# nyu-systems/Grendel-GS

Hardware: AMD Instinct MI355X
Metric: training iters/sec (fwd+bwd) (higher is better)
Workload: dtype f32

## Files before the change

grendel-gs_amd/csrc/binning.hip:

```cpp
#include "common.h"

#include <atomic>
#include <chrono>
#include <cstdlib>
#include <cstring>
#include <mutex>

#include "radix.h"
#ifndef GSR_EMIT_DECODE_BATCH
#define GSR_EMIT_DECODE_BATCH 2
#endif
#include "binning_persist.h"
#include "binning_rows.h"

namespace {

__global__ void __launch_bounds__(SCAN_THREADS)
scan_gather_lookback_kernel(const uint32_t *__restrict__ src, int packed,
                            const uint32_t *__restrict__ idx, uint32_t *__restrict__ out, uint32_t *__restrict__ out2,
                            long long n, unsigned long long *__restrict__ state, uint32_t *__restrict__ ticket, int nb,
                            uint32_t *__restrict__ host_total, uint32_t seq,
                            const unsigned long long *__restrict__ early) {
    __shared__ uint32_t smem[4];
    __shared__ uint32_t s_bid;
// ... 510 lines not shown
}

int prepare_lookback(const PrepCall &c, uint32_t *ticket) {
    const int P = c.P;
    hipStream_t stream = c.stream;
    const PrepLayout L = prep_layout(P, c.width, c.height);
    const int gx = (c.width + GSR_BLOCK_X - 1) / GSR_BLOCK_X, gy = (c.height + GSR_BLOCK_Y - 1) / GSR_BLOCK_Y;
    char *base = reinterpret_cast<char *>(c.prep);
    uint32_t *tt = reinterpret_cast<uint32_t *>(base + L.tt);
    uint32_t *kA = reinterpret_cast<uint32_t *>(base + L.kA), *vA = reinterpret_cast<uint32_t *>(base + L.vA);
    uint32_t *kB = reinterpret_cast<uint32_t *>(base + L.kB), *vB = reinterpret_cast<uint32_t *>(base + L.vB);
    uint32_t *offsets = reinterpret_cast<uint32_t *>(base + L.offsets);
    TileRect *rects = reinterpret_cast<TileRect *>(base + L.rects);
    char *ctrl = base + L.ctrl;

    GSR_HIP(hipMemsetAsync(base + L.early, 0, (L.ctrl - L.early) + L.C.total, stream));
    const RadixPlan plan = radix_plan(0, 32);
    uint32_t *host_total = nullptr;
    uint32_t seq = 0;
    int rc = total_slot(&host_total, &seq);
    if (rc) return rc;
    uint32_t *tile_hist = yx_path(gx, gy) ? reinterpret_cast<uint32_t *>(base + L.thist) : nullptr;
    const int blocks = gsr_div_up(P, TC_THREADS) < TC_BLOCKS ? gsr_div_up(P, TC_THREADS) : TC_BLOCKS;
    hipLaunchKernelGGL(touch_count_kernel, dim3(blocks), dim3(TC_THREADS), 0, stream, P, gx, gy,
                       reinterpret_cast<const float2 *>(c.means2D), c.depths, c.radii,
                       reinterpret_cast<const float4 *>(c.conic_opacity), c.compute_locally, plan, tt, kA, vA, rects,
                       reinterpret_cast<uint32_t *>(ctrl + L.C.ghist), tile_hist,
                       reinterpret_cast<int32_t *>(base + L.hull), tile_hist ? tile_cull_on(gx * gy) : 0,
                       reinterpret_cast<unsigned long long *>(base + L.early), host_total, seq,
                       reinterpret_cast<uint4 *>(c.zero_ptr), c.zero_bytes / 16);
    int in_first = 1;
    rc = radix_sort_pairs(kA, vA, kB, vB, P, plan, ctrl, L.C, &in_first, stream, nullptr);
    if (rc) return rc;
    uint32_t *sorted_ids = in_first ? vA : vB;
    if (!in_first) {
        hipLaunchKernelGGL(copy_u32_kernel, dim3(gsr_div_up(P, GSR_ONE_DIM_BLOCK)), dim3(GSR_ONE_DIM_BLOCK), 0, stream,
                           (long long)P, vB, vA);
        sorted_ids = vA;
    }
    if (g_tie_order.load(std::memory_order_relaxed) == 1)
        hipLaunchKernelGGL(depth_tie_fixup_kernel, dim3(gsr_div_up(P, GSR_ONE_DIM_BLOCK)), dim3(GSR_ONE_DIM_BLOCK), 0,
                           stream, (long long)P, in_first ? kA : kB, sorted_ids,
                           reinterpret_cast<const float2 *>(c.means2D));
    const int nbs = gsr_div_up(P, SCAN_TILE);
    hipLaunchKernelGGL(scan_gather_lookback_kernel, dim3(nbs), dim3(SCAN_THREADS), 0, stream, tt,
                       tile_hist ? 1 : 0, sorted_ids, offsets,
                       reinterpret_cast<uint32_t *>(base + L.segoff), (long long)P,
                       reinterpret_cast<unsigned long long *>(ctrl + L.C.scan_state),
                       reinterpret_cast<uint32_t *>(ctrl + L.C.tickets), nbs, (uint32_t *)nullptr, seq,
                       reinterpret_cast<const unsigned long long *>(base + L.early));
    GSR_LAUNCH_CHECK();
    *ticket = seq;
    return 0;
}

int prepare_persistent(const PrepCall &c, uint32_t *ticket) {
    if (!(persist_effective_mode() & PERSIST_P) || g_tie_order.load(std::memory_order_relaxed) != 0) return 1;
    int dev = 0;
    GSR_HIP(hipGetDevice(&dev));
    if (dev < 0 || dev >= 64) return 1;
    PersistCaps caps;
    persist_caps(dev, &caps);
    const int max_tpw = env_cap("GSR_BIN_MAX_TPW", PP_MAX_TPW + 1) <= PP_MAX_TPW ? env_cap("GSR_BIN_MAX_TPW", PP_MAX_TPW + 1) : 1;
    long long nb = radix_blocks(c.P);
    int items = 4;
    if (nb > caps.grid_p && (nb + 1) / 2 <= caps.grid_p) {
        items = 8;
        nb = (nb + 1) / 2;
    }
    const int G = (int)(nb < caps.grid_p ? nb : caps.grid_p);
    if (G <= 0 || nb > (long long)G * max_tpw) return 1;
    const long long admit = persist_admit(dev, c.stream);
    if (admit < 0) return 1;
    const int P = c.P;
    const PrepLayout L = prep_layout(P, c.width, c.height);
    const PersistLayoutP PL = persist_layout_p(G);
    const int gx = (c.width + GSR_BLOCK_X - 1) / GSR_BLOCK_X, gy = (c.height + GSR_BLOCK_Y - 1) / GSR_BLOCK_Y;
    char *base = reinterpret_cast<char *>(c.prep);
    char *ctrl = base + L.ctrl;
    GSR_HIP(hipMemsetAsync(base + L.early, 0, (L.ctrl - L.early) + PL.zero_bytes, c.stream));
    uint32_t *host_total = nullptr;
    uint32_t seq = 0;
    int rc = total_slot(&host_total, &seq);
    if (rc) return rc;
    PrepPersistArgs a{};
    a.P = P; a.gx = gx; a.gy = gy;
    a.means2D = reinterpret_cast<const float2 *>(c.means2D);
    a.depths = c.depths;
    a.radii = c.radii;
    a.conic_opacity = reinterpret_cast<const float4 *>(c.conic_opacity);
    a.mask = c.compute_locally;
    a.tt = reinterpret_cast<uint32_t *>(base + L.tt);
    a.kA = reinterpret_cast<uint32_t *>(base + L.kA); a.vA = reinterpret_cast<uint32_t *>(base + L.vA);
    a.kB = reinterpret_cast<uint32_t *>(base + L.kB); a.vB = reinterpret_cast<uint32_t *>(base + L.vB);
    a.offsets = reinterpret_cast<uint32_t *>(base + L.offsets);
    a.segoff = reinterpret_cast<uint32_t *>(base + L.segoff);
    a.rects = reinterpret_cast<TileRect *>(base + L.rects);
    a.tile_hist = yx_path(gx, gy) ? reinterpret_cast<uint32_t *>(base + L.thist) : nullptr;
    a.cull = a.tile_hist ? tile_cull_on(gx * gy) : 0;
    a.hull_out = reinterpret_cast<int32_t *>(base + L.hull);
    a.early = reinterpret_cast<unsigned long long *>(base + L.early);
    a.zero16 = reinterpret_cast<uint4 *>(c.zero_ptr);
    a.zero16_n = c.zero_bytes / 16;
    const int ngroups = (G + GB_FAN - 1) / GB_FAN;
    a.sync.leaf = reinterpret_cast<uint32_t *>(ctrl + PL.sync);
    a.sync.root = a.sync.leaf + (size_t)ngroups * GB_LEAF_STRIDE;
    a.sync.flags = a.sync.root + GB_LEAF_STRIDE;
    a.tstamp = timeline_buffer(0, G);
    a.grp = reinterpret_cast<uint32_t *>(ctrl + PL.grp);
    a.cnt = reinterpret_cast<uint32_t *>(ctrl + PL.cnt);
    a.wtot = reinterpret_cast<unsigned long long *>(ctrl + PL.wtot);
    a.host_total = host_total;
    a.seq = seq;
    a.done_word = g_persist_done[dev];
    a.done_seq = (uint32_t)admit;
    a.timeout_ticks = 5000000ull;
    a.force_abort = force_abort_env('p') ? 1 : 0;
    if (items == 4) hipLaunchKernelGGL(bin_prepare_persist_kernel<4>, dim3(G), dim3(PP_THREADS), 0, c.stream, a);
    else hipLaunchKernelGGL(bin_prepare_persist_kernel<8>, dim3(G), dim3(PP_THREADS), 0, c.stream, a);
    GSR_LAUNCH_CHECK();
    *ticket = seq;
    return 0;
}
}

namespace {
int prepare_async_impl(int P, int width, int height, const float *means2D, const float *depths, const int32_t *radii,
                       const float *conic_opacity, const uint8_t *compute_locally, void *prep, size_t prep_bytes,
                       uint32_t *ticket, gsr_stream_t stream_, void *zero_ptr, size_t zero_bytes);
}
extern "C" int gsr_bin_prepare_async(int P, int width, int height, const float *means2D, const float *depths,
                                     const int32_t *radii, const float *conic_opacity, const uint8_t *compute_locally,
                                     void *prep, size_t prep_bytes, uint32_t *ticket, gsr_stream_t stream_) {
    return prepare_async_impl(P, width, height, means2D, depths, radii, conic_opacity, compute_locally, prep, prep_bytes,
                              ticket, stream_, nullptr, 0);
}
namespace {
int prepare_async_impl(int P, int width, int height, const float *means2D, const float *depths, const int32_t *radii,
                       const float *conic_opacity, const uint8_t *compute_locally, void *prep, size_t prep_bytes,
                       uint32_t *ticket, gsr_stream_t stream_, void *zero_ptr, size_t zero_bytes) {
    hipStream_t stream = reinterpret_cast<hipStream_t>(stream_);
    if (P < 0 || width <= 0 || height <= 0 || !ticket) return GSR_EINVAL;
    *ticket = 0;
    if (P == 0) return 0;
    if (!means2D || !depths || !radii || !conic_opacity || !compute_locally || !prep) return GSR_EINVAL;
    if (P > RADIX_MAX_N) return GSR_EINVAL;
    if (prep_bytes < prep_layout_full(P, width, height).total) return GSR_ENOSPACE;
    const int gx = (width + GSR_BLOCK_X - 1) / GSR_BLOCK_X, gy = (height + GSR_BLOCK_Y - 1) / GSR_BLOCK_Y;
    if (gx > 0xFFFF || gy > 0xFFFF) return GSR_EINVAL;
    PrepCall c{P, width, height, means2D, depths, radii, conic_opacity, compute_locally, prep, stream, true,
               zero_ptr, zero_bytes};
    {
        int dev0 = 0;
        GSR_HIP(hipGetDevice(&dev0));
        const int fault = persist_fault_check(dev0);
        if (fault) return fault;
    }
    int rc = prepare_persistent(c, ticket);
    if (rc == 1) {
        c.persistent = false;
        rc = prepare_lookback(c, ticket);
    }
    if (rc) return rc;
    int dev = 0;
// ... 423 lines not shown
```

grendel-gs_amd/csrc/binning_persist.h:

```cpp
#pragma once

namespace {

constexpr int TT_SHIFT = 20;
constexpr uint32_t TT_MASK = (1u << TT_SHIFT) - 1u;
constexpr uint32_t GB_ABORT = 0x80000000u;
constexpr int GB_FAN = 32;
constexpr int GB_LEAF_STRIDE = 32;
constexpr uint32_t PAIRS_ABORTED = 0xFFFFFFFFu;

struct GridSync {
    uint32_t *leaf;
    uint32_t *root;
    uint32_t *flags;
};
__host__ __device__ inline size_t grid_sync_words(int G) {
    return (size_t)(2 * ((G + GB_FAN - 1) / GB_FAN) + 1) * GB_LEAF_STRIDE;
}

__device__ __forceinline__ bool grid_barrier_try_abort(const GridSync gs, uint32_t complete) {
    uint32_t r = __hip_atomic_load(gs.root, __ATOMIC_RELAXED, __HIP_MEMORY_SCOPE_AGENT);
    while (true) {
        if (r & GB_ABORT) return true;
        if (r == complete) return false;
// ... 228 lines not shown
    out.xs = (uint32_t)minx | ((uint32_t)maxx << 16);
    out.ys = (uint32_t)miny | ((uint32_t)maxy << 16);
    out.mask = ~0ull;
    if (!cull || w * h > 64) {
        if (dxy) {
            atomicAdd(&dxy[0][minx], h);
            atomicAdd(&dxy[0][maxx], -h);
            atomicAdd(&dxy[1][miny], w);
            atomicAdd(&dxy[1][maxy], -w);
            atomicAdd(&dxy[2][miny], 1);
            atomicAdd(&dxy[2][maxy], -1);
        }
        return (uint32_t)(w * h);
    }
    const unsigned long long mask = gsr_tile_mask(xy, co, minx, miny, maxx, maxy);
    out.mask = mask;
    if (dxy) {
        const unsigned long long rowm = gsr_full_mask(w);
        int prev_cnt = 0, run_a0 = 0, run_len = 0, run_mult = 0;
        for (int r = 0; r < h; r++) {
            unsigned long long bits = (mask >> (r * w)) & rowm;
            const int cnt = __popcll(bits);
            if (cnt != prev_cnt) atomicAdd(&dxy[1][miny + r], cnt - prev_cnt);
            prev_cnt = cnt;
            while (bits) {
                const int a0 = __ffsll((long long)bits) - 1;
                const unsigned long long rest = ~(bits >> a0);
                const int len = rest ? __ffsll((long long)rest) - 1 : 64 - a0;
                if (run_mult && a0 == run_a0 && len == run_len) {
                    run_mult++;
                } else {
                    if (run_mult) {
                        atomicAdd(&dxy[0][minx + run_a0], run_mult);
                        atomicAdd(&dxy[0][minx + run_a0 + run_len], -run_mult);
                    }
                    run_a0 = a0; run_len = len; run_mult = 1;
                }
                bits &= ~(gsr_full_mask(len) << a0);
            }
        }
        if (run_mult) {
            atomicAdd(&dxy[0][minx + run_a0], run_mult);
            atomicAdd(&dxy[0][minx + run_a0 + run_len], -run_mult);
        }
        if (prev_cnt) atomicAdd(&dxy[1][maxy], -prev_cnt);
    }
    return (uint32_t)__popcll(mask);
}

template <int ITEMS, int THREADS>
struct PersistSmem {
    uint16_t wtab[THREADS / 64][RADIX_DIGITS];
    uint32_t gbase[RADIX_DIGITS];
    uint32_t skey[ITEMS * THREADS], sval[ITEMS * THREADS];
    uint32_t scan_tmp[THREADS / 64];
    unsigned long long scan64[THREADS / 64];
    uint32_t flag;
};

template <int ITEMS, int THREADS>
__device__ __forceinline__ void clear_wtab(PersistSmem<ITEMS, THREADS> &sm) {
    uint32_t *p = reinterpret_cast<uint32_t *>(&sm.wtab[0][0]);
    for (int i = threadIdx.x; i < (THREADS / 64) * RADIX_DIGITS / 2; i += THREADS) p[i] = 0u;
}

template <int ITEMS, int THREADS>
__device__ __forceinline__ void count_wave_digits(PersistSmem<ITEMS, THREADS> &sm, const uint32_t (&key)[ITEMS],
                                                  long long wbase, long long n, int shift, uint32_t mask) {
    const int lane = threadIdx.x & 63, wave = threadIdx.x >> 6;
#pragma unroll
    for (int r = 0; r < ITEMS; r++) {
        if (wbase + r * 64 + lane < n) {
            const uint32_t dg = (key[r] >> shift) & mask;
            atomicAdd(reinterpret_cast<uint32_t *>(sm.wtab[wave]) + (dg >> 1), 1u << (16 * (dg & 1u)));
        }
    }
}

template <int ITEMS, int THREADS>
__device__ __forceinline__ void scatter_rank(PersistSmem<ITEMS, THREADS> &sm, const uint32_t (&key)[ITEMS],
                                             const uint32_t (&val)[ITEMS], long long tbase, long long n, int shift,
                                             int nbits, uint32_t &tot_out, uint32_t &run_out) {
    constexpr int WAVES = THREADS / 64;
    const uint32_t mask = (1u << nbits) - 1u;
    const int lane = threadIdx.x & 63, wave = threadIdx.x >> 6;
    const long long wbase = tbase + (long long)wave * (ITEMS * 64);
    const uint32_t d = threadIdx.x;
    uint32_t cnt[WAVES], tot = 0;
#pragma unroll
    for (int w = 0; w < WAVES; w++) {
        cnt[w] = d < RADIX_DIGITS ? sm.wtab[w][d] : 0u;
        tot += cnt[w];
    }
    uint32_t all;
    uint32_t run = block_exclusive_scan_n<WAVES>(tot, sm.scan_tmp, &all);
    tot_out = tot;
    run_out = run;
    if (d < RADIX_DIGITS) {
#pragma unroll
        for (int w = 0; w < WAVES; w++) {
            sm.wtab[w][d] = (uint16_t)run;
            run += cnt[w];
        }
    }
    __syncthreads();
    const unsigned long long lt = (1ull << lane) - 1ull;
#pragma unroll
    for (int r = 0; r < ITEMS; r++) {
        const bool valid = wbase + r * 64 + lane < n;
        const uint32_t dg = (key[r] >> shift) & mask;
        const unsigned long long m = match_digit(dg, valid, nbits);
        const uint32_t rank = __popcll(m & lt);
        uint16_t *cursor = sm.wtab[wave];
        uint32_t pos = 0;
        if (valid) pos = cursor[dg] + rank;
        asm volatile("" ::: "memory");
        __builtin_amdgcn_wave_barrier();
        if (valid && rank == 0) cursor[dg] = (uint16_t)(pos + (uint32_t)__popcll(m));
        asm volatile("" ::: "memory");
        __builtin_amdgcn_wave_barrier();
        if (valid) {
            sm.skey[pos] = key[r];
            sm.sval[pos] = val[r];
        }
    }
}

template <int ITEMS, int THREADS, bool WT_VALS>
__device__ __forceinline__ void scatter_write(PersistSmem<ITEMS, THREADS> &sm, long long tbase, long long n, int shift,
                                              int nbits, uint32_t first, uint32_t run, uint32_t *__restrict__ keys_out,
                                              uint32_t *__restrict__ vals_out) {
    constexpr int TILE = ITEMS * THREADS;
    const uint32_t mask = (1u << nbits) - 1u;
    if (threadIdx.x < RADIX_DIGITS) sm.gbase[threadIdx.x] = first - run;
    __syncthreads();
    const long long rem = n - tbase;
    const int count = rem < TILE ? (int)rem : TILE;
#pragma unroll
    for (int r = 0; r < ITEMS; r++) {
        const int i = r * THREADS + threadIdx.x;
        if (i < count) {
            const uint32_t k = sm.skey[i];
            const uint32_t dst = sm.gbase[(k >> shift) & mask] + (uint32_t)i;
            st_agent(&keys_out[dst], k);
            if (WT_VALS) st_agent(&vals_out[dst], sm.sval[i]);
            else vals_out[dst] = sm.sval[i];
        }
    }
    __syncthreads();
}

template <int ITEMS, int THREADS, bool WT_VALS>
__device__ __forceinline__ uint32_t scatter_tile(PersistSmem<ITEMS, THREADS> &sm, const uint32_t (&key)[ITEMS],
                                                 const uint32_t (&val)[ITEMS], long long tbase, long long n, int shift,
                                                 int nbits, uint32_t first, uint32_t *__restrict__ keys_out,
                                                 uint32_t *__restrict__ vals_out) {
    uint32_t tot, run;
    scatter_rank(sm, key, val, tbase, n, shift, nbits, tot, run);
    scatter_write<ITEMS, THREADS, WT_VALS>(sm, tbase, n, shift, nbits, first, run, keys_out, vals_out);
    return tot;
}

__device__ __forceinline__ unsigned long long wave_sum64(unsigned long long v) {
#pragma unroll
    for (int d = 32; d >= 1; d >>= 1) v += __shfl_xor(v, d, 64);
    return v;
}

__device__ __forceinline__ uint32_t clamp_pair_count(unsigned long long d) {
    return d >= 0xFFFFFFFEull ? 0xFFFFFFFEu : (uint32_t)d;
}
__device__ __forceinline__ void publish_pair_count(unsigned long long *early, unsigned long long mine, uint32_t nwg,
                                                   uint32_t *host_total, uint32_t seq) {
    __hip_atomic_fetch_add(early, mine, __ATOMIC_RELAXED, __HIP_MEMORY_SCOPE_AGENT);
    uint32_t *ticket = reinterpret_cast<uint32_t *>(early + 1);
    const uint32_t t = __hip_atomic_fetch_add(ticket, 1u, __ATOMIC_ACQ_REL, __HIP_MEMORY_SCOPE_AGENT);
    if (t + 1u == nwg && host_total) {
        const unsigned long long d = __hip_atomic_load(early, __ATOMIC_RELAXED, __HIP_MEMORY_SCOPE_AGENT);
        __hip_atomic_store(host_total, clamp_pair_count(d), __ATOMIC_RELAXED, __HIP_MEMORY_SCOPE_SYSTEM);
        __hip_atomic_store(host_total + 1, seq, __ATOMIC_RELEASE, __HIP_MEMORY_SCOPE_SYSTEM);
    }
}

#define GSR_TS(k)                                                                                       \
    do {                                                                                                \
        if (a.tstamp && threadIdx.x == 0) a.tstamp[(size_t)blockIdx.x * 32 + (k)] = __builtin_amdgcn_s_memrealtime(); \
    } while (0)

constexpr int PP_THREADS = 1024, PP_WAVES = PP_THREADS / 64;
constexpr int PP_MAX_TPW = 8;

struct PrepPersistArgs {
    int P, gx, gy;
    const float2 *means2D;
    const float *depths;
    const int32_t *radii;
    const float4 *conic_opacity;
    const uint8_t *mask;
    uint32_t *tt, *kA, *vA, *kB, *vB, *offsets;
    uint32_t *segoff;
    TileRect *rects;
    uint32_t *tile_hist;
    int cull;
    int32_t *hull_out;
    unsigned long long *early;
    uint4 *zero16;
    size_t zero16_n;
    GridSync sync;
    uint32_t *cnt;
    uint32_t *grp;
    unsigned long long *wtot;
    uint32_t *host_total;
    uint32_t seq;
    uint32_t *done_word;
    uint32_t done_seq;
    uint64_t timeout_ticks;
    int force_abort;
    unsigned long long *tstamp;
};

struct PPExtra {
    int32_t dxy[3][RADIX_DIGITS + 1];
    int s_lo, s_hi;
};


template <int PP_ITEMS>
__global__ void __launch_bounds__(PP_THREADS)
bin_prepare_persist_kernel(const PrepPersistArgs a) {
    constexpr int PP_TILE = PP_THREADS * PP_ITEMS;
    __shared__ PersistSmem<PP_ITEMS, PP_THREADS> sm;
    __shared__ PPExtra ex;
    __shared__ uint32_t red2[2 * PP_THREADS];
    const uint32_t G = gridDim.x, w = blockIdx.x;
    const int lane = threadIdx.x & 63, wave = threadIdx.x >> 6;
    const long long P = a.P;
    const long long nb = (P + PP_TILE - 1) / PP_TILE;
    const long long t0 = (long long)w * nb / G, t1 = (long long)(w + 1) * nb / G;
    const bool keep = (t1 - t0) == 1;
    const uint32_t d = threadIdx.x;
    uint32_t epoch = 0;
    GSR_TS(0);
    uint32_t key[PP_ITEMS], val[PP_ITEMS];
    for (size_t i = (size_t)w * PP_THREADS + threadIdx.x; i < a.zero16_n; i += (size_t)G * PP_THREADS)
        a.zero16[i] = make_uint4(0u, 0u, 0u, 0u);

    if (threadIdx.x <= RADIX_DIGITS) ex.dxy[0][threadIdx.x] = ex.dxy[1][threadIdx.x] = ex.dxy[2][threadIdx.x] = 0;
    if (threadIdx.x == 0) { ex.s_lo = a.gy; ex.s_hi = 0; }
    clear_wtab(sm);
    __syncthreads();
    {
        const int total = a.gx * a.gy;
        const int per = (total + PP_THREADS - 1) / PP_THREADS;
        const int b0 = threadIdx.x * per, b1 = min(b0 + per, total);
        int first = 0x7fffffff, last = -1;
#pragma unroll 8
        for (int b = b0; b < b1; b++) {
            const int on = a.mask[b] != 0;
            first = min(first, on ? b : 0x7fffffff);
            last = max(last, on ? b : -1);
        }
        if (last >= 0) {
            atomicMin(&ex.s_lo, first / a.gx);
            atomicMax(&ex.s_hi, last / a.gx + 1);
        }
    }
    __syncthreads();
    const int hull0 = ex.s_lo, hull1 = ex.s_hi;
    if (w == 0 && threadIdx.x == 0) {
        a.hull_out[0] = hull1 > hull0 ? hull0 : 0;
        a.hull_out[1] = hull1 > hull0 ? hull1 : 0;
    }
    uint32_t mytot = 0;
    unsigned long long nsum = 0;
    for (long long t = t0; t < t1; t++) {
        const long long wbase = t * PP_TILE + (long long)wave * (PP_ITEMS * 64);
#pragma unroll
        for (int r0 = 0; r0 < PP_ITEMS; r0 += 4) {
        int rad[4];
        float2 xy[4];
        float4 co[4];
        float dep[4];
#pragma unroll
        for (int q4 = 0; q4 < 4; q4++) {
            const int r = r0 + q4;
            const long long i = wbase + r * 64 + lane;
            const long long ic = i < P ? i : P - 1;
            rad[q4] = a.radii[ic];
            xy[q4] = a.means2D[ic];
            co[q4] = a.conic_opacity[ic];
            dep[q4] = a.depths[ic];
        }
#pragma unroll
        for (int q4 = 0; q4 < 4; q4++) {
            const int r = r0 + q4;
            const long long i = wbase + r * 64 + lane;
            key[r] = 0xFFFFFFFFu;
            val[r] = (uint32_t)i;
            if (i < P) {
                uint32_t n = 0;
                TileRect rect{0u, 0u, 0ull};
                if (rad[q4] > 0) {
                    float exx, eyy;
                    if (gsr_alpha_extent(co[q4], exx, eyy)) {
                        int minx, miny, maxx, maxy;
                        gsr_get_rect(xy[q4].x, xy[q4].y, rad[q4], a.gx, a.gy, minx, miny, maxx, maxy);
                        minx = max(minx, (int)ceilf((xy[q4].x - exx - (GSR_BLOCK_X - 1)) * (1.0f / GSR_BLOCK_X)));
                        maxx = min(maxx, (int)floorf((xy[q4].x + exx) * (1.0f / GSR_BLOCK_X)) + 1);
                        miny = max(max(miny, hull0), (int)ceilf((xy[q4].y - eyy - (GSR_BLOCK_Y - 1)) * (1.0f / GSR_BLOCK_Y)));
                        maxy = min(min(maxy, hull1), (int)floorf((xy[q4].y + eyy) * (1.0f / GSR_BLOCK_Y)) + 1);
                        if (maxx > minx && maxy > miny)
                            n = gsr_rect_tiles(xy[q4], co[q4], minx, miny, maxx, maxy, a.cull != 0,
                                               a.tile_hist ? ex.dxy : nullptr, rect);
                    }
                }
                if (n) key[r] = __float_as_uint(dep[q4]);
                nsum += n;
                st_agent(&a.tt[i], (a.tile_hist && n) ? (n | (((rect.ys >> 16) - (rect.ys & 0xFFFFu)) << TT_SHIFT)) : n);
                a.rects[i] = rect;
                if (!keep) {
                    st_agent(&a.kA[i], key[r]);
                    st_agent(&a.vA[i], val[r]);
                }
            }
        }
        }
        count_wave_digits(sm, key, wbase, P, 0, 0xFFu);
        __syncthreads();
        if (d < RADIX_DIGITS) {
#pragma unroll
            for (int wv = 0; wv < PP_WAVES; wv++) mytot += sm.wtab[wv][d];
        }
        if (!keep) {
            __syncthreads();
            clear_wtab(sm);
            __syncthreads();
        }
    }
    if (d < RADIX_DIGITS) publish_counts(a.cnt, a.grp, w, d, mytot);
    {
        nsum = wave_sum64(nsum);
        __syncthreads();
        if (lane == 0) sm.scan64[wave] = nsum;
        __syncthreads();
        if (threadIdx.x == 0) {
            unsigned long long tot = 0;
            for (int wv = 0; wv < PP_WAVES; wv++) tot += sm.scan64[wv];
            if (tot) __hip_atomic_fetch_add(a.early, tot, __ATOMIC_RELAXED, __HIP_MEMORY_SCOPE_AGENT);
        }
    }
    if (a.tile_hist) {
        const uint32_t xcc = __builtin_amdgcn_s_getreg(20 | (3 << 11)) & 7u;
        for (int p = 0; p < 3; p++) {
            const uint32_t v = threadIdx.x < RADIX_DIGITS ? (uint32_t)ex.dxy[p][threadIdx.x] : 0u;
            uint32_t all;
            const uint32_t c = block_exclusive_scan_n<PP_WAVES>(v, sm.scan_tmp, &all) + v;
            if (threadIdx.x < RADIX_DIGITS && c)
                __hip_atomic_fetch_add(&a.tile_hist[(xcc * RADIX_MAX_PASSES + p) * RADIX_DIGITS + threadIdx.x], c,
                                       __ATOMIC_RELAXED, __HIP_MEMORY_SCOPE_WORKGROUP);
        }
    }
    GSR_TS(1);
    if (!grid_barrier(a.sync, G, epoch, a.timeout_ticks, &sm.flag, a.force_abort != 0)) {
        if (threadIdx.x == 0) {
            a.offsets[P] = PAIRS_ABORTED;
            __hip_atomic_store(a.host_total, PAIRS_ABORTED, __ATOMIC_RELAXED, __HIP_MEMORY_SCOPE_SYSTEM);
            __hip_atomic_store(a.host_total + 1, a.seq, __ATOMIC_RELEASE, __HIP_MEMORY_SCOPE_SYSTEM);
            if (a.done_seq) __hip_atomic_store(a.done_word, a.done_seq, __ATOMIC_RELEASE, __HIP_MEMORY_SCOPE_SYSTEM);
        }
        return;
    }
    GSR_TS(2);
    if (w == 0 && threadIdx.x == 0) {
        const unsigned long long dsum = __hip_atomic_load(a.early, __ATOMIC_RELAXED, __HIP_MEMORY_SCOPE_AGENT);
        __hip_atomic_store(a.host_total, clamp_pair_count(dsum), __ATOMIC_RELAXED, __HIP_MEMORY_SCOPE_SYSTEM);
        __hip_atomic_store(a.host_total + 1, a.seq, __ATOMIC_RELEASE, __HIP_MEMORY_SCOPE_SYSTEM);
    }
    const uint64_t forever = 100000000ull;
    const uint32_t ngroups = (G + GB_FAN - 1) / GB_FAN;
    for (int p = 0; p < 4; p++) {
        const int shift = 8 * p;
        uint32_t *const ksrc = (p & 1) ? a.kB : a.kA, *const vsrc = (p & 1) ? a.vB : a.vA;
        uint32_t *const kdst = (p & 1) ? a.kA : a.kB, *const vdst = (p & 1) ? a.vA : a.vB;
        const uint32_t *const cnt_p = a.cnt + (size_t)p * G * RADIX_DIGITS;
        const uint32_t *const grp_p = a.grp + (size_t)p * ngroups * RADIX_DIGITS;
        uint32_t before, total, all, first;
        if (keep && counts_fit_registers<PP_THREADS>(G)) {
            CountLoads cl;
            counts_issue<PP_THREADS>(cnt_p, grp_p, G, w, cl);
            uint32_t tot, run;
            scatter_rank(sm, key, val, t0 * PP_TILE, P, shift, 8, tot, run);
            counts_finish<PP_THREADS>(cl, w, reinterpret_cast<uint32_t *>(red2), before, total);
            first = block_exclusive_scan_n<PP_WAVES>(total, sm.scan_tmp, &all) + before;
            scatter_write<PP_ITEMS, PP_THREADS, true>(sm, t0 * PP_TILE, P, shift, 8, first, run, kdst, vdst);
        } else {
        counts_before<PP_THREADS>(cnt_p, grp_p, G, w, sm.skey, before, total);
        first = block_exclusive_scan_n<PP_WAVES>(total, sm.scan_tmp, &all) + before;
        for (long long t = t0; t < t1; t++) {
            const long long tbase = t * PP_TILE;
            const long long wbase = tbase + (long long)wave * (PP_ITEMS * 64);
            if (!keep) {
#pragma unroll
                for (int r = 0; r < PP_ITEMS; r++) {
                    const long long j = wbase + r * 64 + lane;
                    key[r] = j < P ? ld_agent(&ksrc[j]) : 0xFFFFFFFFu;
                    val[r] = j < P ? ld_agent(&vsrc[j]) : 0u;
                }
                count_wave_digits(sm, key, wbase, P, shift, 0xFFu);
                __syncthreads();
            }
            first += scatter_tile<PP_ITEMS, PP_THREADS, true>(sm, key, val, tbase, P, shift, 8, first, kdst, vdst);
            if (!keep) {
                clear_wtab(sm);
                __syncthreads();
            }
        }
        }
        GSR_TS(3 + 4 * p);
        if (!grid_barrier(a.sync, G, epoch, forever, &sm.flag)) { barrier_fault(a.done_word, 0x100u + epoch); return; }
        GSR_TS(4 + 4 * p);
        if (p == 3) break;
        if (keep) {
            clear_wtab(sm);
            __syncthreads();
        }
        mytot = 0;
        for (long long t = t0; t < t1; t++) {
            const long long wbase = t * PP_TILE + (long long)wave * (PP_ITEMS * 64);
#pragma unroll
            for (int r = 0; r < PP_ITEMS; r++) {
                const long long j = wbase + r * 64 + lane;
                key[r] = j < P ? ld_agent(&kdst[j]) : 0xFFFFFFFFu;
                val[r] = j < P ? ld_agent(&vdst[j]) : 0u;
            }
            count_wave_digits(sm, key, wbase, P, shift + 8, 0xFFu);
            __syncthreads();
            if (d < RADIX_DIGITS) {
#pragma unroll
                for (int wv = 0; wv < PP_WAVES; wv++) mytot += sm.wtab[wv][d];
            }
            if (!keep) {
                __syncthreads();
                clear_wtab(sm);
                __syncthreads();
            }
// ... 409 lines not shown
            count_wave_digits(sm, key, wbase, s1, a.xbits, ymask);
            __syncthreads();
            first += scatter_tile<PS_ITEMS, PS_THREADS, false>(sm, key, val, tbase, s1, a.xbits, a.ybits, first, a.kA, a.point_list);
            clear_wtab(sm);
            __syncthreads();
        }
    }
    GSR_TS(7);
    if (solo) solo_sync();
    else if (!grid_barrier(a.sync, G, epoch, forever, &sm.flag)) { barrier_fault(a.done_word, 0x200u + epoch); return; }
    GSR_TS(8);
    if (w == 0 && threadIdx.x == 0 && a.done_seq)
        __hip_atomic_store(a.done_word, a.done_seq, __ATOMIC_RELEASE, __HIP_MEMORY_SCOPE_SYSTEM);
    {
        int2 *const ranges = reinterpret_cast<int2 *>(a.ranges);
        auto load6 = [&](long long j, uint32_t (&k)[6]) {
            k[0] = j > 0 ? ld_agent(&a.kA[j - 1]) : 0xFFFFFFFFu;
            if (j + 4 <= D) {
                const unsigned long long q0 = ld_agent64(reinterpret_cast<const unsigned long long *>(a.kA + j));
                const unsigned long long q1 = ld_agent64(reinterpret_cast<const unsigned long long *>(a.kA + j + 2));
                k[1] = (uint32_t)q0; k[2] = (uint32_t)(q0 >> 32); k[3] = (uint32_t)q1; k[4] = (uint32_t)(q1 >> 32);
            } else {
#pragma unroll
                for (int i = 0; i < 4; i++) k[1 + i] = j + i < D ? ld_agent(&a.kA[j + i]) : 0xFFFFFFFFu;
            }
            k[5] = j + 4 < D ? ld_agent(&a.kA[j + 4]) : 0xFFFFFFFFu;
        };
        long long j = s0 + (long long)threadIdx.x * 4;
        uint32_t k[6], kn[6];
        if (j < s1) load6(j, k);
        while (j < s1) {
            const long long jn = j + PS_THREADS * 4;
            if (jn < s1) load6(jn, kn);
#pragma unroll
            for (int i = 1; i <= 4; i++) {
                if (j + i - 1 >= D) break;
                const uint32_t kk = k[i];
                if (k[i - 1] != kk || k[i + 1] != kk) {
                    const uint32_t tl = (kk >> a.xbits) * (uint32_t)a.gx + (kk & xmask);
                    if (!a.mask[tl]) continue;
                    if (k[i - 1] != kk) st_agent(reinterpret_cast<uint32_t *>(&ranges[tl].x), (uint32_t)(j + i - 1));
                    if (k[i + 1] != kk) st_agent(reinterpret_cast<uint32_t *>(&ranges[tl].y), (uint32_t)(j + i));
                }
            }
#pragma unroll
            for (int i = 0; i < 6; i++) k[i] = kn[i];
            j = jn;
        }
    }
    GSR_TS(9);
}

struct PersistLayoutP {
    size_t sync, grp, cnt, wtot, zero_bytes, total;
};
inline PersistLayoutP persist_layout_p(int G) {
    PersistLayoutP L;
    const int ngroups = (G + GB_FAN - 1) / GB_FAN;
    size_t o = 0;
    L.sync = o; o += align_up(sizeof(uint32_t) * grid_sync_words(G));
    L.grp = o; o += align_up(sizeof(uint32_t) * 4 * (size_t)ngroups * RADIX_DIGITS);
    L.zero_bytes = o;
    L.cnt = o; o += align_up(sizeof(uint32_t) * 4 * (size_t)G * RADIX_DIGITS);
    L.wtot = o; o += align_up(sizeof(unsigned long long) * (size_t)G);
    L.total = o;
    return L;
}
struct PersistLayoutS {
    size_t sync, grp, grp_solo, cnt, cnt_solo, zero_bytes, total;
};
inline PersistLayoutS persist_layout_s(int G) {
    PersistLayoutS L;
    const int ngroups = (G + GB_FAN - 1) / GB_FAN;
    size_t o = 0;
    L.sync = o; o += align_up(sizeof(uint32_t) * grid_sync_words(G));
    L.grp = o; o += align_up(sizeof(uint32_t) * 2 * (size_t)ngroups * RADIX_DIGITS);
    L.grp_solo = o; o += align_up(sizeof(uint32_t) * 2 * RADIX_DIGITS);
    L.zero_bytes = o;
    L.cnt = o; o += align_up(sizeof(uint32_t) * 2 * (size_t)G * RADIX_DIGITS);
    L.cnt_solo = o; o += align_up(sizeof(uint32_t) * 2 * RADIX_DIGITS);
    L.total = o;
    return L;
}
constexpr int PERSIST_MAX_GRID_P = 1024;
constexpr int PERSIST_MAX_GRID_S = 4096;
constexpr long long PERSIST_SORT_MAX_PAIRS = 6ll << 20;

struct PersistCaps {
    int grid_p = 0, grid_s = 0;
    bool init = false;
};
std::mutex g_persist_mutex;
PersistCaps g_persist_caps[64];
uint32_t *g_persist_done[64] = {};
uint32_t g_persist_faults_seen[64] = {};
uint32_t g_persist_solo_seen[64] = {};
int g_persist_backoff[64] = {};
bool g_persist_faulted[64] = {};
uint32_t g_persist_seq[64] = {};
hipStream_t g_persist_stream[64] = {};
bool g_persist_any[64] = {};

enum { PERSIST_OFF = 0, PERSIST_P = 1, PERSIST_S = 2 };
int persist_mode() {
    static const int mode = [] {
        const char *e = getenv("GSR_BIN_PERSIST");
        if (!e || !*e || strcmp(e, "1") == 0) return PERSIST_P | PERSIST_S;
        if (strcmp(e, "p") == 0) return (int)PERSIST_P;
        if (strcmp(e, "s") == 0) return (int)PERSIST_S;
        return (int)PERSIST_OFF;
    }();
    return mode;
}
std::atomic<int> g_persist_override{-1};

unsigned long long *g_timeline[2] = {nullptr, nullptr};
int g_timeline_grid[2] = {0, 0};
unsigned long long *timeline_buffer(int which, int G) {
    static const bool on = [] { const char *e = getenv("GSR_BIN_TIMELINE"); return e && *e == '1'; }();
    if (!on) return nullptr;
    if (!g_timeline[which]) {
        void *p = nullptr;
        if (hipMalloc(&p, sizeof(unsigned long long) * 32 * PERSIST_MAX_GRID_S) != hipSuccess) return nullptr;
        g_timeline[which] = reinterpret_cast<unsigned long long *>(p);
    }
    (void)hipMemset(g_timeline[which], 0, sizeof(unsigned long long) * 32 * (size_t)G);
    g_timeline_grid[which] = G;
    return g_timeline[which];
}

int env_cap(const char *name, int dflt) {
    const char *e = getenv(name);
    if (!e || !*e) return dflt;
    const int v = atoi(e);
    return v > 0 && v < dflt ? v : dflt;
}

int persist_caps(int dev, PersistCaps *out) {
    std::lock_guard<std::mutex> guard(g_persist_mutex);
    PersistCaps &c = g_persist_caps[dev];
    if (!c.init) {
        c.init = true;
        int cus = 0, per_p = 0, per_p8 = 0, per_s = 0;
        if (hipDeviceGetAttribute(&cus, hipDeviceAttributeMultiprocessorCount, dev) == hipSuccess && cus > 0 &&
            hipOccupancyMaxActiveBlocksPerMultiprocessor(&per_p, bin_prepare_persist_kernel<4>, PP_THREADS, 0) == hipSuccess &&
            hipOccupancyMaxActiveBlocksPerMultiprocessor(&per_p8, bin_prepare_persist_kernel<8>, PP_THREADS, 0) == hipSuccess &&
            hipOccupancyMaxActiveBlocksPerMultiprocessor(&per_s, bin_sort_persist_kernel, PS_THREADS, 0) == hipSuccess) {
            c.grid_p = (per_p >= 1 && per_p8 >= 1) ? (cus < PERSIST_MAX_GRID_P ? cus : PERSIST_MAX_GRID_P) : 0;
            const long long gs = (long long)cus * (per_s < 4 ? per_s : 4);
            c.grid_s = per_s >= 1 ? (int)(gs < PERSIST_MAX_GRID_S ? gs : PERSIST_MAX_GRID_S) : 0;
        }
        void *p = nullptr;
        if (hipHostMalloc(&p, 64, hipHostMallocDefault) == hipSuccess) {
            memset(p, 0, 64);
            g_persist_done[dev] = reinterpret_cast<uint32_t *>(p);
        } else {
            c.grid_p = c.grid_s = 0;
        }
        (void)hipGetLastError();
    }
    *out = c;
    out->grid_p = env_cap("GSR_BIN_GRID_P", c.grid_p);
    out->grid_s = env_cap("GSR_BIN_GRID_S", c.grid_s);
    return 0;
}

long long persist_admit(int dev, hipStream_t stream) {
    hipStreamCaptureStatus cs = hipStreamCaptureStatusNone;
    if (hipStreamIsCapturing(stream, &cs) == hipSuccess && cs != hipStreamCaptureStatusNone) return 0;
    (void)hipGetLastError();
    std::lock_guard<std::mutex> guard(g_persist_mutex);
    if (g_persist_faulted[dev]) return -1;
    if (g_persist_any[dev] && g_persist_stream[dev] != stream) {
// ... 47 lines not shown
```

Baseline: 777.3.

## Replace four-pass LSD depth radix sort with histogram-based bucket sort in persistent kernel

In the persistent binning prepare kernel, when each block owns exactly one tile, depth keys are first distributed into up to 255 buckets. The bucket boundaries come from a global 4096-bin histogram over the observed key range. Each block then sorts its own bucket locally in shared memory and computes offsets directly, replacing the four global LSD radix passes and their grid barriers. The original path is kept as a fallback if any bucket exceeds block capacity. This adds extra grid barriers, global histogram atomics, and more shared memory, plus minor tweaks to the wave reductions and to register hints.

After: 786.4, median of 6. +1.2%, better.

```diff
diff --git a/grendel-gs_amd/csrc/binning.hip b/grendel-gs_amd/csrc/binning.hip
--- a/grendel-gs_amd/csrc/binning.hip
+++ b/grendel-gs_amd/csrc/binning.hip
@@ -586,6 +586,11 @@
     GSR_LAUNCH_CHECK();
     *ticket = seq;
     return 0;
+}
+
+bool depth_buckets_on() {
+    const char *e = getenv("GSR_BIN_DEPTH_SORT");
+    return !(e && strcmp(e, "lsd") == 0);
 }
 
 int prepare_persistent(const PrepCall &c, uint32_t *ticket) {
@@ -644,6 +649,8 @@
     a.grp = reinterpret_cast<uint32_t *>(ctrl + PL.grp);
     a.cnt = reinterpret_cast<uint32_t *>(ctrl + PL.cnt);
     a.wtot = reinterpret_cast<unsigned long long *>(ctrl + PL.wtot);
+    a.bins = reinterpret_cast<uint32_t *>(ctrl + PL.bins);
+    a.depth_buckets = depth_buckets_on() ? 1 : 0;
     a.host_total = host_total;
     a.seq = seq;
     a.done_word = g_persist_done[dev];
diff --git a/grendel-gs_amd/csrc/binning_persist.h b/grendel-gs_amd/csrc/binning_persist.h
--- a/grendel-gs_amd/csrc/binning_persist.h
+++ b/grendel-gs_amd/csrc/binning_persist.h
@@ -304,10 +304,10 @@
 struct PersistSmem {
     uint16_t wtab[THREADS / 64][RADIX_DIGITS];
     uint32_t gbase[RADIX_DIGITS];
+    unsigned long long scan64[THREADS / 64];
+    uint32_t scan_tmp[THREADS / 64];
+    uint32_t flag;
     uint32_t skey[ITEMS * THREADS], sval[ITEMS * THREADS];
-    uint32_t scan_tmp[THREADS / 64];
-    unsigned long long scan64[THREADS / 64];
-    uint32_t flag;
 };
 
 template <int ITEMS, int THREADS>
@@ -316,25 +316,45 @@
     for (int i = threadIdx.x; i < (THREADS / 64) * RADIX_DIGITS / 2; i += THREADS) p[i] = 0u;
 }
 
+struct ByteDigit {
+    int shift;
+    uint32_t mask;
+    __device__ __forceinline__ uint32_t operator()(uint32_t k) const { return (k >> shift) & mask; }
+};
+constexpr int BK_BINS = 4096, BK_BIN_BITS = 12;
+constexpr uint32_t BK_TAIL = 255u;
+struct BucketDigit {
+    const uint8_t *map;
+    uint32_t kmin;
+    int sh;
+    __device__ __forceinline__ uint32_t operator()(uint32_t k) const {
+        return k == 0xFFFFFFFFu ? BK_TAIL : (uint32_t)map[(k - kmin) >> sh];
+    }
+};
+
+template <int ITEMS, int THREADS, class DG>
+__device__ __forceinline__ void count_wave_digits(PersistSmem<ITEMS, THREADS> &sm, const uint32_t (&key)[ITEMS],
+                                                  long long wbase, long long n, const DG digit) {
+    const int lane = threadIdx.x & 63, wave = threadIdx.x >> 6;
+#pragma unroll
+    for (int r = 0; r < ITEMS; r++) {
+        if (wbase + r * 64 + lane < n) {
+            const uint32_t dg = digit(key[r]);
+            atomicAdd(reinterpret_cast<uint32_t *>(sm.wtab[wave]) + (dg >> 1), 1u << (16 * (dg & 1u)));
+        }
+    }
+}
 template <int ITEMS, int THREADS>
 __device__ __forceinline__ void count_wave_digits(PersistSmem<ITEMS, THREADS> &sm, const uint32_t (&key)[ITEMS],
                                                   long long wbase, long long n, int shift, uint32_t mask) {
-    const int lane = threadIdx.x & 63, wave = threadIdx.x >> 6;
-#pragma unroll
-    for (int r = 0; r < ITEMS; r++) {
-        if (wbase + r * 64 + lane < n) {
-            const uint32_t dg = (key[r] >> shift) & mask;
-            atomicAdd(reinterpret_cast<uint32_t *>(sm.wtab[wave]) + (dg >> 1), 1u << (16 * (dg & 1u)));
-        }
-    }
-}
-
-template <int ITEMS, int THREADS>
+    count_wave_digits(sm, key, wbase, n, ByteDigit{shift, mask});
+}
+
+template <int ITEMS, int THREADS, class DG>
 __device__ __forceinline__ void scatter_rank(PersistSmem<ITEMS, THREADS> &sm, const uint32_t (&key)[ITEMS],
-                                             const uint32_t (&val)[ITEMS], long long tbase, long long n, int shift,
+                                             const uint32_t (&val)[ITEMS], long long tbase, long long n, const DG digit,
                                              int nbits, uint32_t &tot_out, uint32_t &run_out) {
     constexpr int WAVES = THREADS / 64;
-    const uint32_t mask = (1u << nbits) - 1u;
     const int lane = threadIdx.x & 63, wave = threadIdx.x >> 6;
     const long long wbase = tbase + (long long)wave * (ITEMS * 64);
     const uint32_t d = threadIdx.x;
@@ -360,7 +380,7 @@
 #pragma unroll
     for (int r = 0; r < ITEMS; r++) {
         const bool valid = wbase + r * 64 + lane < n;
-        const uint32_t dg = (key[r] >> shift) & mask;
+        const uint32_t dg = digit(key[r]);
         const unsigned long long m = match_digit(dg, valid, nbits);
         const uint32_t rank = __popcll(m & lt);
         uint16_t *cursor = sm.wtab[wave];
@@ -378,6 +398,13 @@
     }
 }
 
+template <int ITEMS, int THREADS>
+__device__ __forceinline__ void scatter_rank(PersistSmem<ITEMS, THREADS> &sm, const uint32_t (&key)[ITEMS],
+                                             const uint32_t (&val)[ITEMS], long long tbase, long long n, int shift,
+                                             int nbits, uint32_t &tot_out, uint32_t &run_out) {
+    scatter_rank(sm, key, val, tbase, n, ByteDigit{shift, (1u << nbits) - 1u}, nbits, tot_out, run_out);
+}
+
 template <int ITEMS, int THREADS, bool WT_VALS>
 __device__ __forceinline__ void scatter_write(PersistSmem<ITEMS, THREADS> &sm, long long tbase, long long n, int shift,
                                               int nbits, uint32_t first, uint32_t run, uint32_t *__restrict__ keys_out,
@@ -416,6 +443,22 @@
 __device__ __forceinline__ unsigned long long wave_sum64(unsigned long long v) {
 #pragma unroll
     for (int d = 32; d >= 1; d >>= 1) v += __shfl_xor(v, d, 64);
+    return v;
+}
+
+__device__ __forceinline__ uint32_t xor_lane(uint32_t v, int lane, int d) {
+    return (uint32_t)__builtin_amdgcn_ds_bpermute((lane ^ d) << 2, (int)v);
+}
+__device__ __forceinline__ int opaque_lane() {
+    int lane = threadIdx.x & 63;
+    asm volatile("" : "+v"(lane));
+    return lane;
+}
+__device__ __forceinline__ unsigned long long wave_sum64_local(unsigned long long v) {
+    const int lane = opaque_lane();
+#pragma unroll
+    for (int d = 32; d >= 1; d >>= 1)
+        v += (unsigned long long)xor_lane((uint32_t)v, lane, d) | ((unsigned long long)xor_lane((uint32_t)(v >> 32), lane, d) << 32);
     return v;
 }
 
@@ -462,6 +505,8 @@
     uint32_t *cnt;
     uint32_t *grp;
     unsigned long long *wtot;
+    uint32_t *bins;
+    int depth_buckets;
     uint32_t *host_total;
     uint32_t seq;
     uint32_t *done_word;
@@ -476,13 +521,122 @@
     int s_lo, s_hi;
 };
 
+constexpr int BK_ITEMS = 8;
+constexpr int BK_CAP = BK_ITEMS * PP_THREADS;
+constexpr int BK_PASS = RADIX_MAX_PASSES;
+struct PPBucket {
+    uint8_t map[BK_BINS];
+    uint32_t lo, n, live;
+};
+
+template <int ITEMS, int THREADS>
+__device__ __forceinline__ void bucket_scatter_write(PersistSmem<ITEMS, THREADS> &sm, long long n, const BucketDigit digit,
+                                                     uint32_t first, uint32_t run, uint32_t *__restrict__ keys_out,
+                                                     uint32_t *__restrict__ vals_out, uint32_t *__restrict__ ids_out) {
+    constexpr int TILE = ITEMS * THREADS;
+    if (threadIdx.x < RADIX_DIGITS) sm.gbase[threadIdx.x] = first - run;
+    __syncthreads();
+    const int count = n < TILE ? (int)n : TILE;
+#pragma unroll
+    for (int r = 0; r < ITEMS; r++) {
+        const int i = r * THREADS + threadIdx.x;
+        if (i < count) {
+            const uint32_t k = sm.skey[i];
+            const uint32_t dg = digit(k);
+            const uint32_t dst = sm.gbase[dg] + (uint32_t)i;
+            if (dg == BK_TAIL) {
+                ids_out[dst] = sm.sval[i];
+            } else {
+                st_agent(&keys_out[dst], k);
+                st_agent(&vals_out[dst], sm.sval[i]);
+            }
+        }
+    }
+    __syncthreads();
+}
+
+template <int THREADS>
+__device__ __forceinline__ void bucket_sort_span(PersistSmem<BK_ITEMS, THREADS> &s, const uint32_t *__restrict__ kin,
+                                                 const uint32_t *__restrict__ vin, uint32_t lo, uint32_t n,
+                                                 uint32_t *__restrict__ red) {
+    constexpr int WAVES = THREADS / 64;
+    const int lane = threadIdx.x & 63, wave = threadIdx.x >> 6;
+    const uint32_t wbase = (uint32_t)wave * (BK_ITEMS * 64);
+    uint32_t key[BK_ITEMS], val[BK_ITEMS];
+    uint32_t mn = 0xFFFFFFFFu, mx = 0u;
+#pragma unroll
+    for (int r = 0; r < BK_ITEMS; r++) {
+        const uint32_t i = wbase + r * 64 + lane;
+        key[r] = i < n ? ld_agent(&kin[lo + i]) : 0xFFFFFFFFu;
+        val[r] = i < n ? ld_agent(&vin[lo + i]) : 0u;
+    }
+#pragma unroll
+    for (int r = 0; r < BK_ITEMS; r++) {
+        if (wbase + r * 64 + lane < n) {
+            mn = min(mn, key[r]);
+            mx = max(mx, key[r]);
+        }
+    }
+#pragma unroll
+    for (int d = 32; d >= 1; d >>= 1) {
+        mn = min(mn, (uint32_t)__shfl_xor(mn, d, 64));
+        mx = max(mx, (uint32_t)__shfl_xor(mx, d, 64));
+    }
+    if (lane == 0) {
+        red[wave] = mn;
+        red[WAVES + wave] = mx;
+    }
+    __syncthreads();
+#pragma unroll
+    for (int wv = 0; wv < WAVES; wv++) {
+        mn = min(mn, red[wv]);
+        mx = max(mx, red[WAVES + wv]);
+    }
+    const uint32_t diff = mx > mn ? mx - mn : 0u;
+    const int nbits = diff ? 32 - __clz(diff) : 0;
+#pragma unroll
+    for (int r = 0; r < BK_ITEMS; r++) key[r] -= mn;
+    if (nbits == 0) {
+#pragma unroll
+        for (int r = 0; r < BK_ITEMS; r++) {
+            const uint32_t i = wbase + r * 64 + lane;
+            if (i < n) s.sval[i] = val[r];
+        }
+        __syncthreads();
+        return;
+    }
+    const int passes = (nbits + 7) / 8, pb = (nbits + passes - 1) / passes;
+    for (int shift = 0; shift < nbits; shift += pb) {
+        clear_wtab(s);
+        __syncthreads();
+        count_wave_digits(s, key, (long long)wbase, (long long)n, shift, (1u << pb) - 1u);
+        __syncthreads();
+        uint32_t tot, run;
+        scatter_rank(s, key, val, 0ll, (long long)n, shift, pb, tot, run);
+        __syncthreads();
+        if (shift + pb < nbits) {
+#pragma unroll
+            for (int r = 0; r < BK_ITEMS; r++) {
+                const uint32_t i = wbase + r * 64 + lane;
+                if (i < n) {
+                    key[r] = s.skey[i];
+                    val[r] = s.sval[i];
+                }
+            }
+            __syncthreads();
+        }
+    }
+}
+
 
 template <int PP_ITEMS>
 __global__ void __launch_bounds__(PP_THREADS)
 bin_prepare_persist_kernel(const PrepPersistArgs a) {
     constexpr int PP_TILE = PP_THREADS * PP_ITEMS;
-    __shared__ PersistSmem<PP_ITEMS, PP_THREADS> sm;
+    __shared__ PersistSmem<BK_ITEMS, PP_THREADS> sm8;
+    PersistSmem<PP_ITEMS, PP_THREADS> &sm = *reinterpret_cast<PersistSmem<PP_ITEMS, PP_THREADS> *>(&sm8);
     __shared__ PPExtra ex;
+    __shared__ PPBucket bk;
     __shared__ uint32_t red2[2 * PP_THREADS];
     const uint32_t G = gridDim.x, w = blockIdx.x;
     const int lane = threadIdx.x & 63, wave = threadIdx.x >> 6;
@@ -490,6 +644,7 @@
     const long long nb = (P + PP_TILE - 1) / PP_TILE;
     const long long t0 = (long long)w * nb / G, t1 = (long long)(w + 1) * nb / G;
     const bool keep = (t1 - t0) == 1;
+    const bool try_buckets = a.depth_buckets && nb == (long long)G && counts_fit_registers<PP_THREADS>(G);
     const uint32_t d = threadIdx.x;
     uint32_t epoch = 0;
     GSR_TS(0);
@@ -525,6 +680,7 @@
     }
     uint32_t mytot = 0;
     unsigned long long nsum = 0;
+    uint32_t kmn = 0xFFFFFFFFu, kmx = 0u;
     for (long long t = t0; t < t1; t++) {
         const long long wbase = t * PP_TILE + (long long)wave * (PP_ITEMS * 64);
 #pragma unroll
@@ -566,7 +722,11 @@
                                                a.tile_hist ? ex.dxy : nullptr, rect);
                     }
                 }
-                if (n) key[r] = __float_as_uint(dep[q4]);
+                if (n) {
+                    key[r] = __float_as_uint(dep[q4]);
+                    kmn = min(kmn, key[r]);
+                    kmx = max(kmx, key[r]);
+                }
                 nsum += n;
                 st_agent(&a.tt[i], (a.tile_hist && n) ? (n | (((rect.ys >> 16) - (rect.ys & 0xFFFFu)) << TT_SHIFT)) : n);
                 a.rects[i] = rect;
@@ -577,6 +737,7 @@
             }
         }
         }
+        if (try_buckets) continue;
         count_wave_digits(sm, key, wbase, P, 0, 0xFFu);
         __syncthreads();
         if (d < RADIX_DIGITS) {
@@ -589,16 +750,36 @@
             __syncthreads();
         }
     }
-    if (d < RADIX_DIGITS) publish_counts(a.cnt, a.grp, w, d, mytot);
+    if (!try_buckets && d < RADIX_DIGITS) publish_counts(a.cnt, a.grp, w, d, mytot);
     {
-        nsum = wave_sum64(nsum);
+        nsum = wave_sum64_local(nsum);
+        {
+            const int ol = opaque_lane();
+#pragma unroll
+            for (int o = 32; o >= 1; o >>= 1) {
+                kmn = min(kmn, xor_lane(kmn, ol, o));
+                kmx = max(kmx, xor_lane(kmx, ol, o));
+            }
+        }
         __syncthreads();
-        if (lane == 0) sm.scan64[wave] = nsum;
+        if (lane == 0) {
+            sm.scan64[wave] = nsum;
+            red2[wave] = kmn;
+            red2[PP_WAVES + wave] = kmx;
+        }
         __syncthreads();
         if (threadIdx.x == 0) {
             unsigned long long tot = 0;
-            for (int wv = 0; wv < PP_WAVES; wv++) tot += sm.scan64[wv];
+            for (int wv = 0; wv < PP_WAVES; wv++) {
+                tot += sm.scan64[wv];
+                kmn = min(kmn, red2[wv]);
+                kmx = max(kmx, red2[PP_WAVES + wv]);
+            }
             if (tot) __hip_atomic_fetch_add(a.early, tot, __ATOMIC_RELAXED, __HIP_MEMORY_SCOPE_AGENT);
+            if (try_buckets && kmn <= kmx) {
+                __hip_atomic_fetch_max(&a.bins[BK_BINS], ~kmn, __ATOMIC_RELAXED, __HIP_MEMORY_SCOPE_AGENT);
+                __hip_atomic_fetch_max(&a.bins[BK_BINS + 1], kmx, __ATOMIC_RELAXED, __HIP_MEMORY_SCOPE_AGENT);
+            }
         }
     }
     if (a.tile_hist) {
@@ -630,6 +811,170 @@
     }
     const uint64_t forever = 100000000ull;
     const uint32_t ngroups = (G + GB_FAN - 1) / GB_FAN;
+    if (try_buckets) {
+        static_assert(BK_BINS == 4 * PP_THREADS, "four bins per thread");
+        const long long wbase0 = t0 * PP_TILE + (long long)wave * (PP_ITEMS * 64);
+        const uint32_t kmin = ~ld_agent(&a.bins[BK_BINS]), kmax = ld_agent(&a.bins[BK_BINS + 1]);
+        const uint32_t NB = min(G, BK_TAIL);
+        bool buckets = kmin <= kmax && kmax != 0xFFFFFFFFu;
+        if (buckets) {
+            const uint32_t range = kmax - kmin;
+            const int sh = max((range ? 32 - __clz(range) : 0) - BK_BIN_BITS, 0);
+            const BucketDigit digit{bk.map, kmin, sh};
+            uint32_t *const lbin = sm8.skey;
+            for (int i = threadIdx.x; i < BK_BINS; i += PP_THREADS) lbin[i] = 0u;
+            __syncthreads();
+#pragma unroll
+            for (int r = 0; r < PP_ITEMS; r++)
+                if (key[r] != 0xFFFFFFFFu) atomicAdd(&lbin[(key[r] - kmin) >> sh], 1u);
+            __syncthreads();
+            for (int i = threadIdx.x; i < BK_BINS; i += PP_THREADS) {
+                const uint32_t c = lbin[i];
+                if (c) __hip_atomic_fetch_add(&a.bins[i], c, __ATOMIC_RELAXED, __HIP_MEMORY_SCOPE_AGENT);
+            }
+            GSR_TS(21);
+            if (!grid_barrier(a.sync, G, epoch, forever, &sm.flag)) { barrier_fault(a.done_word, 0x200u + epoch); return; }
+            GSR_TS(22);
+            {
+                uint32_t c4[4], s4 = 0, live;
+#pragma unroll
+                for (int k = 0; k < 4; k++) {
+                    c4[k] = ld_agent(&a.bins[threadIdx.x * 4 + k]);
+                    s4 += c4[k];
+                }
+                uint32_t start = block_exclusive_scan_n<PP_WAVES>(s4, sm.scan_tmp, &live);
+#pragma unroll
+                for (int k = 0; k < 4; k++) {
+                    bk.map[threadIdx.x * 4 + k] = (uint8_t)(start * NB / live);
+                    start += c4[k];
+                }
+            }
+            __syncthreads();
+            count_wave_digits(sm, key, wbase0, P, digit);
+            __syncthreads();
+            if (d < RADIX_DIGITS) {
+                mytot = 0;
+#pragma unroll
+                for (int wv = 0; wv < PP_WAVES; wv++) mytot += sm.wtab[wv][d];
+                publish_counts(a.cnt + (size_t)BK_PASS * G * RADIX_DIGITS, a.grp + (size_t)BK_PASS * ngroups * RADIX_DIGITS, w,
+                               d, mytot);
+            }
+            GSR_TS(23);
+            if (!grid_barrier(a.sync, G, epoch, forever, &sm.flag)) { barrier_fault(a.done_word, 0x200u + epoch); return; }
+            GSR_TS(24);
+            uint32_t tot, run, before, total, all;
+            counts_before<PP_THREADS>(a.cnt + (size_t)BK_PASS * G * RADIX_DIGITS,
+                                      a.grp + (size_t)BK_PASS * ngroups * RADIX_DIGITS, G, w,
+                                      reinterpret_cast<uint32_t *>(red2), before, total);
+            if (__syncthreads_or(d < BK_TAIL && total > (uint32_t)BK_CAP)) {
+                buckets = false;
+            } else {
+                scatter_rank(sm, key, val, t0 * PP_TILE, P, digit, 8, tot, run);
+                const uint32_t dstart = block_exclusive_scan_n<PP_WAVES>(total, sm.scan_tmp, &all);
+                if (d == w) {
+                    bk.lo = dstart;
+                    bk.n = w < NB ? total : 0u;
+                }
+                if (d == BK_TAIL) bk.live = dstart;
+                bucket_scatter_write(sm, P - t0 * PP_TILE, digit, dstart + before, run, a.kB, a.vB, a.vA);
+            }
+        }
+        if (buckets) {
+            GSR_TS(25);
+            if (!grid_barrier(a.sync, G, epoch, forever, &sm.flag)) { barrier_fault(a.done_word, 0x200u + epoch); return; }
+            GSR_TS(26);
+            const uint32_t lo = bk.lo, n = bk.n, live = bk.live;
+            bucket_sort_span<PP_THREADS>(sm8, a.kB, a.vB, lo, n, reinterpret_cast<uint32_t *>(red2));
+#pragma unroll
+            for (int r = 0; r < BK_ITEMS; r++) {
+                const uint32_t i = r * PP_THREADS + threadIdx.x;
+                if (i < n) a.vA[lo + i] = sm8.sval[i];
+            }
+            uint32_t v[BK_ITEMS], hv[BK_ITEMS], s = 0, sh2 = 0;
+#pragma unroll
+            for (int k = 0; k < BK_ITEMS; k++) {
+                const uint32_t i = threadIdx.x * BK_ITEMS + k;
+                const uint32_t x = i < n ? ld_agent(&a.tt[sm8.sval[i]]) : 0u;
+                v[k] = a.tile_hist ? (x & TT_MASK) : x;
+                hv[k] = a.tile_hist ? (x >> TT_SHIFT) : 0u;
+                s += v[k];
+                sh2 += hv[k];
+            }
+            unsigned long long wsum = wave_sum64((unsigned long long)s | ((unsigned long long)sh2 << 32));
+            if (lane == 0) sm.scan64[wave] = wsum;
+            __syncthreads();
+            if (threadIdx.x == 0) {
+                unsigned long long tot = 0;
+                for (int wv = 0; wv < PP_WAVES; wv++) tot += sm.scan64[wv];
+                st_agent64(&a.wtot[w], tot);
+            }
+            GSR_TS(27);
+            if (!grid_barrier(a.sync, G, epoch, forever, &sm.flag)) { barrier_fault(a.done_word, 0x200u + epoch); return; }
+            GSR_TS(28);
+            if (w == 0 && threadIdx.x == 0 && a.done_seq)
+                __hip_atomic_store(a.done_word, a.done_seq, __ATOMIC_RELEASE, __HIP_MEMORY_SCOPE_SYSTEM);
+            unsigned long long carry, gtot;
+            {
+                unsigned long long x = 0, y = 0;
+                for (uint32_t k = threadIdx.x; k < G; k += PP_THREADS) {
+                    const unsigned long long t = ld_agent64(&a.wtot[k]);
+                    y += t;
+                    if (k < w) x += t;
+                }
+                x = wave_sum64(x);
+                y = wave_sum64(y);
+                __syncthreads();
+                if (lane == 0) {
+                    sm.scan64[wave] = x;
+                    reinterpret_cast<unsigned long long *>(red2)[wave] = y;
+                }
+                __syncthreads();
+                carry = gtot = 0;
+                for (int wv = 0; wv < PP_WAVES; wv++) {
+                    carry += sm.scan64[wv];
+                    gtot += reinterpret_cast<unsigned long long *>(red2)[wv];
+                }
+            }
+            uint32_t tots, toth;
+            const uint32_t local = block_exclusive_scan_n<PP_WAVES>(s, sm.scan_tmp, &tots);
+            const uint32_t localh = block_exclusive_scan_n<PP_WAVES>(sh2, sm.scan_tmp, &toth);
+            uint32_t runp = (uint32_t)carry + local, runh = (uint32_t)(carry >> 32) + localh;
+#pragma unroll
+            for (int k = 0; k < BK_ITEMS; k++) {
+                const uint32_t i = threadIdx.x * BK_ITEMS + k;
+                if (i < n) {
+                    a.offsets[lo + i] = runp;
+                    a.segoff[lo + i] = runh;
+                }
+                runp += v[k];
+                runh += hv[k];
+            }
+            for (long long j = (long long)live + (long long)w * PP_THREADS + threadIdx.x; j < P; j += (long long)G * PP_THREADS) {
+                a.offsets[j] = (uint32_t)gtot;
+                a.segoff[j] = (uint32_t)(gtot >> 32);
+            }
+            if (w == G - 1 && threadIdx.x == 0) {
+                a.offsets[P] = clamp_pair_count(__hip_atomic_load(a.early, __ATOMIC_RELAXED, __HIP_MEMORY_SCOPE_AGENT));
+                a.segoff[P] = (uint32_t)(gtot >> 32);
+            }
+            GSR_TS(31);
+            return;
+        }
+        __syncthreads();
+        clear_wtab(sm);
+        __syncthreads();
+        count_wave_digits(sm, key, wbase0, P, 0, 0xFFu);
+        __syncthreads();
+        if (d < RADIX_DIGITS) {
+            mytot = 0;
+#pragma unroll
+            for (int wv = 0; wv < PP_WAVES; wv++) mytot += sm.wtab[wv][d];
+            publish_counts(a.cnt, a.grp, w, d, mytot);
+        }
+        GSR_TS(17);
+        if (!grid_barrier(a.sync, G, epoch, forever, &sm.flag)) { barrier_fault(a.done_word, 0x200u + epoch); return; }
+        GSR_TS(18);
+    }
     for (int p = 0; p < 4; p++) {
         const int shift = 8 * p;
         uint32_t *const ksrc = (p & 1) ? a.kB : a.kA, *const vsrc = (p & 1) ? a.vB : a.vA;
@@ -638,11 +983,13 @@
         const uint32_t *const grp_p = a.grp + (size_t)p * ngroups * RADIX_DIGITS;
         uint32_t before, total, all, first;
         if (keep && counts_fit_registers<PP_THREADS>(G)) {
+            uint32_t wp = w;
+            asm volatile("" : "+s"(wp));
             CountLoads cl;
-            counts_issue<PP_THREADS>(cnt_p, grp_p, G, w, cl);
+            counts_issue<PP_THREADS>(cnt_p, grp_p, G, wp, cl);
             uint32_t tot, run;
             scatter_rank(sm, key, val, t0 * PP_TILE, P, shift, 8, tot, run);
-            counts_finish<PP_THREADS>(cl, w, reinterpret_cast<uint32_t *>(red2), before, total);
+            counts_finish<PP_THREADS>(cl, wp, reinterpret_cast<uint32_t *>(red2), before, total);
             first = block_exclusive_scan_n<PP_WAVES>(total, sm.scan_tmp, &all) + before;
             scatter_write<PP_ITEMS, PP_THREADS, true>(sm, t0 * PP_TILE, P, shift, 8, first, run, kdst, vdst);
         } else {
@@ -1158,16 +1505,17 @@
 }
 
 struct PersistLayoutP {
-    size_t sync, grp, cnt, wtot, zero_bytes, total;
+    size_t sync, grp, bins, cnt, wtot, zero_bytes, total;
 };
 inline PersistLayoutP persist_layout_p(int G) {
     PersistLayoutP L;
     const int ngroups = (G + GB_FAN - 1) / GB_FAN;
     size_t o = 0;
     L.sync = o; o += align_up(sizeof(uint32_t) * grid_sync_words(G));
-    L.grp = o; o += align_up(sizeof(uint32_t) * 4 * (size_t)ngroups * RADIX_DIGITS);
+    L.grp = o; o += align_up(sizeof(uint32_t) * (BK_PASS + 1) * (size_t)ngroups * RADIX_DIGITS);
+    L.bins = o; o += align_up(sizeof(uint32_t) * (BK_BINS + 2));
     L.zero_bytes = o;
-    L.cnt = o; o += align_up(sizeof(uint32_t) * 4 * (size_t)G * RADIX_DIGITS);
+    L.cnt = o; o += align_up(sizeof(uint32_t) * (BK_PASS + 1) * (size_t)G * RADIX_DIGITS);
     L.wtot = o; o += align_up(sizeof(unsigned long long) * (size_t)G);
     L.total = o;
     return L;
@@ -1223,8 +1571,8 @@
 unsigned long long *g_timeline[2] = {nullptr, nullptr};
 int g_timeline_grid[2] = {0, 0};
 unsigned long long *timeline_buffer(int which, int G) {
-    static const bool on = [] { const char *e = getenv("GSR_BIN_TIMELINE"); return e && *e == '1'; }();
-    if (!on) return nullptr;
+    const char *e = getenv("GSR_BIN_TIMELINE");
+    if (!(e && *e == '1')) return nullptr;
     if (!g_timeline[which]) {
         void *p = nullptr;
         if (hipMalloc(&p, sizeof(unsigned long long) * 32 * PERSIST_MAX_GRID_S) != hipSuccess) return nullptr;
```
